# HENDRIX-ZT2/pyaudiorestoration

Measured on AMD Instinct MI355X. Metric: Msamples/sec resampled (192 kHz varispeed), higher is better.
Workload: dtype f32 near taps, far taps (|n| >= 3) as float16 hi + lo x 2^-12 filter banks on v_mfma_f32_16x16x32_f16 with f32 accumulation / f64 positions

## Files before the change

pyaudiorestoration_amd/csrc/sinc2.hip:

```cpp
#define PAR_WANT_BANK2 1
#include "par_common.h"
#include "pos_plan.h"
#include "sinc_taps_gen.h"
#include "sinc_common.h"
#include "sinc_block.h"
#include <algorithm>
#include <atomic>
#include <limits.h>
#include <type_traits>

constexpr int kMaxTilesPerWave = 23;
#ifndef PAR_S2_EXP
#define PAR_S2_EXP 0
#endif

namespace par {

typedef _Float16 half8v __attribute__((ext_vector_type(8)));
typedef _Float16 half2v __attribute__((ext_vector_type(2)));
typedef float float4v __attribute__((ext_vector_type(4)));

constexpr int kRing = 512;
constexpr int kPass = 128;
constexpr float kImgScale = 1024.0f, kImgScaleInv = 0.0009765625f;
constexpr float kImgMax = 32.0f;
constexpr float kQuiet = 0.0001220703125f;


#if PAR_S2_EXP & 64
__device__ unsigned long long* g_s2_phase;
#define S2_MARK(k)                                              \
  do {                                                          \
    const unsigned long long now_ = __builtin_readcyclecounter(); \
    ph_[k] += now_ - pt_;                                       \
    pt_ = now_;                                                 \
  } while (0)
#else
#define S2_MARK(k) do { } while (0)
#endif

struct S2Args {
  int64_t len_out;
  const float* sig;
  int64_t len_in;
  float* out;
  const TileHdr* hdr;
  const BlockRec* rec;
  const BlockRec2* rec2;
  int* redo_count;
  int* redo_list;
  int tiles;
  int tiles_tail;
  int64_t n_big;
  int64_t n_full;
  int64_t n_tiles;
  int n_edge;
  int64_t out_stride;
  FusedArgs fa;
// ... 77 lines not shown
  const bool last = (unsigned)u == ((m >> kRecLastShift) & 63u);
  const float frac = fmaf(u2f, e2, fmaf(uf, e1, F));
  const float e = fmaf(e2, last ? tw0 : tw1, e1);
  const float ri = rintf(frac);
  S2Row o;
  o.s = frac - ri;
  o.c = cbase + irel + (int)ri;
  o.ep = __builtin_amdgcn_fmed3f(e, 0.0f, 3.0e38f);
  o.bad = (m & (kRecSlow0 | kRecSlow1 | kRecCubic)) != 0u || !(fabsf(fabsf(o.s) - 0.5f) > tolf);
  return o;
}


constexpr int kRingF = 1024;
constexpr int kRingH = 512;

template <int NCH, bool MOM = true>
struct S3Lds {
  static constexpr bool kMoments = MOM;
  float ring_head[4 * NCH];
  float ring[kRingF * NCH];
  float ring_tail[4 * NCH];
  _Float16 img[2 * NCH][kRingH];
  float4v qa[kPass];
  float4v qm0[MOM ? kPass : kPass / 4];
  float4v qm1[MOM ? kPass : 1];
  __device__ __forceinline__ float& e2d2(int sl) {
    return MOM ? reinterpret_cast<float*>(&qm0[sl])[3] : reinterpret_cast<float*>(&qm0[0])[sl];
  }
  __device__ __forceinline__ const float& e2d2(int sl) const {
    return MOM ? reinterpret_cast<const float*>(&qm0[sl])[3] : reinterpret_cast<const float*>(&qm0[0])[sl];
  }
#ifdef PAR_S3_LDS_PAD
  uint4 pad[PAR_S3_LDS_PAD / 16];
#endif
  uint4 recs[4][16];
};
static_assert(offsetof(S3Lds<1>, img) % 16 == 0 && offsetof(S3Lds<1>, qa) % 16 == 0 && offsetof(S3Lds<1>, recs) % 16 == 0, "16-byte aligned");
static_assert(offsetof(S3Lds<2>, ring) % 16 == 0 && offsetof(S3Lds<2>, img) % 16 == 0 && offsetof(S3Lds<2>, qa) % 16 == 0 &&
              offsetof(S3Lds<2>, recs) % 16 == 0, "16-byte aligned");
static_assert(sizeof(S3Lds<2>) <= 20480, "eight stereo streams per compute unit (160 KB of LDS)");
using S3LdsUnity = S3Lds<1, false>;
static_assert(sizeof(S3LdsUnity) <= 10240 && offsetof(S3LdsUnity, recs) % 16 == 0 && offsetof(S3LdsUnity, qa) % 16 == 0,
              "sixteen fc = 1 streams per compute unit");

struct S3Pass {
  int c[2];
  float s[2], ep[2];
  int nok[2];
  int j, ws;
};

constexpr int kCtabUnity = 10;
template <bool MOMENTS, bool SIX = true, class LDS>
__device__ __forceinline__ void bank_image3m(LDS& L, const half8v (&fr)[kBank2Frags], const half8v (&fmr)[kBank3Frags],
                                             const int offs, const int l, const int ch = 0) {
  const int bb = l & 15, g = l >> 4;
  const int i0 = offs + 8 * bb + 8 * g;
  half8v xh[3], xl[3];
#pragma unroll
  for (int ks = 0; ks < 3; ++ks) {
    const int ix = (i0 + 32 * ks) & (kRingH - 1);
    xh[ks] = *reinterpret_cast<const half8v*>(&L.img[2 * ch][ix]);
    xl[ks] = *reinterpret_cast<const half8v*>(&L.img[2 * ch + 1][ix]);
  }
  auto frag = [&](int f) { return f < kCtabUnity ? fr[f] : fmr[f - kCtabUnity]; };
  const float4v z = {0.0f, 0.0f, 0.0f, 0.0f};
  float4v e0 = z, lo = z, e1 = z, e2 = z;
#pragma unroll
  for (int ks = 0; ks < 3; ++ks) {
    const half8v f0 = frag(ks);
    e0 = __builtin_amdgcn_mfma_f32_16x16x32_f16(f0, xh[ks], e0, 0, 0, 0);
    lo = __builtin_amdgcn_mfma_f32_16x16x32_f16(frag(5 + ks), xh[ks], lo, 0, 0, 0);
    lo = __builtin_amdgcn_mfma_f32_16x16x32_f16(f0, xl[ks], lo, 0, 0, 0);
    if (ks < 2) {
      const half8v f1 = frag(3 + ks);
      e1 = __builtin_amdgcn_mfma_f32_16x16x32_f16(f1, xh[ks], e1, 0, 0, 0);
      e2 = __builtin_amdgcn_mfma_f32_16x16x32_f16(frag(8 + ks), xh[ks], e2, 0, 0, 0);
    }
  }
  float lo_inv = kBank2LoInv;
  asm volatile("" : "+v"(lo_inv));
  const float4v v0 = e0 + lo * lo_inv, v1 = e1;
  float4v a01 = z, l01 = z, a23 = z, a45 = z, a6 = z;
  if (MOMENTS) {
#pragma unroll
    for (int ks = 0; ks < 3; ++ks) {
      const half8v f01 = frag(kCtabUnity + ks);
      a01 = __builtin_amdgcn_mfma_f32_16x16x32_f16(f01, xh[ks], a01, 0, 0, 0);
      l01 = __builtin_amdgcn_mfma_f32_16x16x32_f16(frag(kCtabUnity + 3 + ks), xh[ks], l01, 0, 0, 0);
      l01 = __builtin_amdgcn_mfma_f32_16x16x32_f16(f01, xl[ks], l01, 0, 0, 0);
      a23 = __builtin_amdgcn_mfma_f32_16x16x32_f16(frag(kCtabUnity + 6 + ks), xh[ks], a23, 0, 0, 0);
      a45 = __builtin_amdgcn_mfma_f32_16x16x32_f16(frag(kCtabUnity + 9 + ks), xh[ks], a45, 0, 0, 0);
      if constexpr (SIX) a6 = __builtin_amdgcn_mfma_f32_16x16x32_f16(frag(kCtabUnity + 12 + ks), xh[ks], a6, 0, 0, 0);
    }
  }
  const float4v m01 = a01 + l01 * lo_inv;
#pragma unroll
  for (int p = 0; p < 2; ++p) {
    const int sl = (8 * bb + 2 * g + p) ^ (bb & 7);
    const float4v row = {v0[2 * p], v0[2 * p + 1], v1[2 * p], v1[2 * p + 1]};
    L.qa[sl] = row;
    const float e2d2 = __uint_as_float(pack_h2(e2[2 * p] * 0.015625f, e2[2 * p + 1] * 0.015625f));
    if constexpr (MOMENTS) {
      const float4v r0 = {m01[2 * p], m01[2 * p + 1], a23[2 * p], e2d2};
      L.qm0[sl] = r0;
      const float4v r1 = {a23[2 * p + 1], a45[2 * p], a45[2 * p + 1], a6[2 * p]};
      L.qm1[sl] = r1;
    } else {
      L.e2d2(sl) = e2d2;
    }
  }
}

template <int MODE, int NCH = 1, class LDS>
__device__ __forceinline__ float s3_out_row(const LDS& L, const int ci, const float sr, const float epr, const int wsK, const int ch = 0) {
  using T32 = TapTab<32>;
  constexpr float kUs = kBank2ScaleInv * kImgScaleInv;
  constexpr float kMs = kImgScaleInv;
  const int sl = ci ^ ((ci >> 3) & 7);
  const int rc = (wsK + ci) & (kRingF - 1);
  const float* xp = &L.ring[NCH * rc + ch];
  const float xm2 = xp[-2 * NCH], xm1 = xp[-NCH], x0 = xp[0], xp1 = xp[NCH], xp2 = xp[2 * NCH];
  const float q = sr * sr, q64 = 64.0f * q;
  const float R1 = fast_rcp(fmaf(q, T32::B[1], T32::A[1])), R2 = fast_rcp(fmaf(q, T32::B[2], T32::A[2]));
  {
    const float E1 = xp1 + xm1, D1 = xp1 - xm1, E2 = xp2 + xm2, D2 = xp2 - xm2;
    const float4v row = L.qa[sl];
    float4v M0 = {0.0f, 0.0f, 0.0f, 0.0f};
    unsigned w2;
    if constexpr (MODE != 1) {
      M0 = L.qm0[sl];
      w2 = __float_as_uint(M0[3]);
    } else {
      w2 = __float_as_uint(L.e2d2(sl));
    }
    const float e = fmaf(q, fmaf(q64, h_lo(w2), row[2]), row[0]), d = fmaf(q, fmaf(q64, h_hi(w2), row[3]), row[1]);
    const float en = fmaf(E2, R2, -(E1 * R1));
    const float dn = fmaf(D2 + D2, R2, -(D1 * R1));
    const float et = fmaf(e, kUs, en), dt = fmaf(d, kUs, dn);
    const float spq = sinpi_poly(q);
    const float unity = spq * fmaf(-sr, fmaf(sr, et, dt), x0 * 0.318309886f);
    if constexpr (MODE == 1) return unity;
    else {
    const float4v Mh = L.qm1[sl];
    const float m3 = Mh[0], m4 = Mh[1], m5 = Mh[2], m6 = Mh[3];
    const float g = epr * fast_rcp(1.0f + epr);
    const float G = 3.14159265f * g, w = G * sr, w2m = w * w, G32 = 32.0f * G;
    float re, im;
    if constexpr (MODE == 3) {
      re = m6 * (1.98412698e-4f * kMs);
      im = 0.0f;
    } else {
      re = m5 * (1.38888889e-3f * kMs);
      im = m5 * (w * -(1.19047619e-3f * kMs));
    }
#define S3_MOM_STEP(Mi, A0, A1, B0)                                   \
    {                                                                 \
      const float al_ = (A1) != 0.0f ? fmaf(w2m, -((A1) * kMs), (A0) * kMs) : (A0) * kMs, be_ = w * -((B0) * kMs);       \
      const float nre_ = fmaf(-G32, im, (Mi) * al_), nim_ = fmaf(G32, re, (Mi) * be_); \
      re = nre_;                                                      \
      im = nim_;                                                      \
    }
    if constexpr (MODE == 3) S3_MOM_STEP(m5, 1.38888889e-3f, 0.0f, 1.19047619e-3f)
    S3_MOM_STEP(m4, 8.33333333e-3f, 0.0f, 6.94444444e-3f)
    S3_MOM_STEP(m3, 4.16666667e-2f, 0.0f, 3.33333333e-2f)
    S3_MOM_STEP(M0[2], 1.66666667e-1f, 5.0e-2f, 1.25e-1f)
    S3_MOM_STEP(M0[1], 0.5f, 0.125f, 3.33333333e-1f)
    S3_MOM_STEP(M0[0], 1.0f, 1.66666667e-1f, 0.5f)
#undef S3_MOM_STEP
    const float S = sr * spq, C = __builtin_amdgcn_cosf(0.5f * sr);
    return fmaf(-g, fmaf(C, re, -(S * im)), unity);
    }
  }
}

template <class LDS>
__device__ __forceinline__ bool s3_convert(LDS& L, const int chunk, const int l) {
  const int wi = chunk * kPass + 2 * l;
  const int ix = wi & (kRingF - 1), ih = wi & (kRingH - 1);
  const float2 xx = *reinterpret_cast<const float2*>(&L.ring[ix]);
  const float x0 = xx.x, x1 = xx.y;
  const float am = fmaxf(fabsf(x0), fabsf(x1));
  const bool ok = !(__ballot(!(fabsf(x0) < kImgMax) || !(fabsf(x1) < kImgMax)) != 0ull ||
                    (__ballot(am >= kQuiet) == 0ull && __ballot(am > 0.0f) != 0ull));
  if ((chunk & 7) == 0 && l < 2) *reinterpret_cast<float2*>(&L.ring_tail[ix]) = xx;
  if ((chunk & 7) == 7 && l == kWave - 1) *reinterpret_cast<float2*>(&L.ring_head[2]) = xx;
  const float s0 = x0 * kImgScale, s1 = x1 * kImgScale;
  const half2v h = {S2_HI(s0), S2_HI(s1)};
  const half2v lo = {(_Float16)((s0 - (float)h[0]) * 4096.0f), (_Float16)((s1 - (float)h[1]) * 4096.0f)};
  *reinterpret_cast<half2v*>(&L.img[0][ih]) = h;
  *reinterpret_cast<half2v*>(&L.img[1][ih]) = lo;
  return ok;
}

template <class LDS>
__device__ __forceinline__ bool s3_convert_ch(LDS& L, const int chunk, const int l, const int ch, const bool mirrors) {
  const int wi = chunk * kPass + 2 * l;
  const int ix = wi & (kRingF - 1), ih = wi & (kRingH - 1);
  const float4v xx = *reinterpret_cast<const float4v*>(&L.ring[2 * ix]);
  const float x0 = ch ? xx[1] : xx[0], x1 = ch ? xx[3] : xx[2];
  const float am = fmaxf(fabsf(x0), fabsf(x1));
  const bool ok = !(__ballot(!(fabsf(x0) < kImgMax) || !(fabsf(x1) < kImgMax)) != 0ull ||
                    (__ballot(am >= kQuiet) == 0ull && __ballot(am > 0.0f) != 0ull));
  if (mirrors) {
    if ((chunk & 7) == 0 && l < 2) *reinterpret_cast<float4v*>(&L.ring_tail[2 * ix]) = xx;
    if ((chunk & 7) == 7 && l == kWave - 1) *reinterpret_cast<float4v*>(&L.ring_head[4]) = xx;
  }
  const float s0 = x0 * kImgScale, s1 = x1 * kImgScale;
  const half2v h = {S2_HI(s0), S2_HI(s1)};
  const half2v lo = {(_Float16)((s0 - (float)h[0]) * 4096.0f), (_Float16)((s1 - (float)h[1]) * 4096.0f)};
  *reinterpret_cast<half2v*>(&L.img[2 * ch][ih]) = h;
  *reinterpret_cast<half2v*>(&L.img[2 * ch + 1][ih]) = lo;
  return ok;
}

constexpr float kEpMaxMom = 0.0125f / (1.0f - 0.0125f);
constexpr float kEpMom5 = 0.0105f / (1.0f - 0.0105f), kEpMom5Lo = 0.95f * kEpMom5;
#ifndef PAR_S3_SHARE_OUT
#define PAR_S3_SHARE_OUT 1
#endif
#ifndef PAR_S3_PIN_MONO
#define PAR_S3_PIN_MONO 0
#endif
template <int NCH, int KIND>
__device__ __forceinline__ void sinc_pipe_body(const S2Args& a, const int bx, S3Lds<NCH, KIND != 1>& L) {
  static_assert(NCH == 1 || NCH == 2, "mono, or an interleaved stereo file");
  static_assert(KIND == 0 || KIND == 3 || NCH == 1, "the stereo form takes every stream");
  static_assert(KIND != 3 || NCH == 2, "one channel of FRAMES");
  constexpr bool kPick = KIND == 3;
  constexpr bool kTwo = NCH == 2 && !kPick;
  constexpr bool kMom = KIND != 1;
  const int l = threadIdx.x & (kWave - 1);
  if (bx < a.n_edge) {
    if constexpr (KIND == 1) return;
    else {
    const int e = bx / kEdgeWavesPerTile, w = bx % kEdgeWavesPerTile;
    const int64_t T = e == 0 ? 0 : a.n_full - 3 + e;
    const int64_t jw = T * kSincTileOutputs + (int64_t)w * kEdgeWaveOut;
    const int nrem = (int)(a.len_out - jw < (int64_t)kEdgeWaveOut ? (a.len_out - jw > 0 ? a.len_out - jw : 0) : kEdgeWaveOut);
    float* const piece = reinterpret_cast<float*>(&L);
    static_assert(sizeof(L) >= fused_capw(2 * NCH, NCH) * NCH * sizeof(float), "the wave's span fits the stream's LDS");
    if constexpr (kPick) {
      static_assert(sizeof(L) >= fused_capw(2, 1) * sizeof(float), "the wave's span fits the stream's LDS");
      if (nrem > 0)
        fused_wave<1, 32, 2, false>(a.len_out, a.sig, nullptr, 2, a.len_in, 32, a.tab, a.tmd, a.out, nullptr, a.out_stride, a.fa, piece, l,
                                    jw, nrem, piece);
      return;
    }
    if (nrem == kEdgeWaveOut)
      fused_wave<NCH, 32, 2 * NCH, true>(a.len_out, a.sig, a.sig + 1, NCH, a.len_in, 32, a.tab, a.tmd, a.out, a.out + 1, NCH, a.fa, piece, l,
                                         jw, nrem, piece);
    else if (nrem > 0)
      fused_wave<NCH, 32, 2 * NCH, false>(a.len_out, a.sig, a.sig + 1, NCH, a.len_in, 32, a.tab, a.tmd, a.out, a.out + 1, NCH, a.fa, piece, l,
                                          jw, nrem, piece);
    return;
    }
  }
  const int64_t stream_id = (int64_t)bx - a.n_edge;
  const int my_tiles = stream_id < a.n_big ? a.tiles : a.tiles_tail;
  const int64_t Ta = stream_id < a.n_big ? stream_id * a.tiles : a.n_big * a.tiles + (stream_id - a.n_big) * a.tiles_tail;
  if (Ta >= a.n_full) return;
  const int64_t Tb = Ta + my_tiles < a.n_full ? Ta + my_tiles : a.n_full;
  const int64_t Ja = Ta * kSincTileOutputs, Jb = Tb * kSincTileOutputs;
  long long A0;
  int hd_dA, hd_fl;
  {
    const int64_t Ti = Ta + l < a.n_tiles ? Ta + l : a.n_tiles - 1;
    const TileHdr h = a.hdr[l <= my_tiles ? Ti : Ta];
    A0 = (long long)(((unsigned long long)(unsigned)__builtin_amdgcn_readfirstlane((int)((unsigned long long)h.anchor >> 32)) << 32) |
                     (unsigned)__builtin_amdgcn_readfirstlane((int)(unsigned)(unsigned long long)h.anchor));
    const long long d = h.anchor - A0;
    hd_fl = h.flags | ((d > -0x40000000ll && d < 0x40000000ll) ? 0 : 1);
    if (a.n_edge > 0 && (Ta + l == 0 || Ta + l >= a.n_full - 2)) hd_fl |= 1 | kTileEdge;
    hd_dA = (int)d;
    if constexpr (KIND == 1 || KIND == 2) {
      const bool any_slow = __ballot(l < my_tiles && Ta + l < Tb && (h.flags & kTileMaySlow) != 0) != 0ull;
      if (any_slow != (KIND == 2)) return;
    }
  }
  half8v fr[kBank2Frags];
  {
    const uint4* src = reinterpret_cast<const uint4*>(kBank2Frags32) + l;
#pragma unroll
    for (int f = 0; f < kBank2Frags; ++f) fr[f] = __builtin_bit_cast(half8v, src[f * kWave]);
// ... 8 lines not shown
    uint4* z = reinterpret_cast<uint4*>(&L.img[0][0]);
    const uint4 zero = {0u, 0u, 0u, 0u};
#pragma unroll
    for (int i = 0; i < (int)(sizeof(L.img) / 16 / kWave); ++i) z[i * kWave + l] = zero;
  }
  const float tolf = (float)((fabs((double)A0) + 2.0e7) * 1.2e-16 + 2.0e-10) + 2.0e-7f;
  const int nJ = (int)(Jb - Ja);
  float* const outW = a.out + (kPick ? a.out_stride : (int64_t)NCH) * Ja;
  const uint4* const recW = reinterpret_cast<const uint4*>(a.rec) + (Ja >> kRecShift);
  const uint4* const rec2W = reinterpret_cast<const uint4*>(a.rec2) + (Ja >> kRecShift);
  const int blk_max = (int)(((a.len_out + kRec - 1) >> kRecShift) - (Ja >> kRecShift)) - 1;

  int j0 = 0;
  int wbase = 0, conv_next = 0, conv_lo = 0, dma_next = 0, dma_bad = INT_MAX, mode = 0, pk = 0;
  int regime = 1;
  int rbA = 0, rbB = 0, rbC = 0;

  const uint4* const rec_lane = (l < 8 ? recW : rec2W) + (l & 7);
  auto fetch_records = [&](int buf, int blk0) {
    if (l < 16) dma_dwordx4(rec_lane + (blk0 < 0 ? 0 : blk0), &L.recs[buf][0]);
  };
  int dma_klo = 0, dma_khi = -1;
  const float* ring_src = a.sig;
  auto ring_restart = [&]() {
    const long long o = A0 + wbase;
    ring_src = a.sig + NCH * o;
    const long long klo = o >= 0 ? 0 : (-o + kPass - 1) / kPass, khi = ((long long)a.len_in - (kPick ? 1 : 0) - o) / kPass - 1;
    dma_klo = (int)(klo > 0x3fffffff ? 0x3fffffff : klo);
    dma_khi = (int)(khi > 0x3fffffff ? 0x3fffffff : (khi < -1 ? -1 : khi));
  };
  const unsigned lane_bytes = 4u * (unsigned)l;
  auto chunk_dma = [&](int k) {
    const bool inside = k >= dma_klo && k <= dma_khi;
    if (!inside) dma_bad = k < dma_bad ? k : dma_bad;
    const float* src = inside ? ring_src + (long long)(kPass * NCH) * k : a.sig;
    if constexpr (NCH == 2) dma_chunk256(src, lane_bytes, &L.ring[(k & 7) * (kPass * 2)]);
    else dma_chunk128(src, lane_bytes, &L.ring[(k & 7) * kPass]);
  };
  auto push_tile = [&](int64_t T) {
    if (l == 0) {
      const int slot = atomicAdd(a.redo_count, 1);
      a.redo_list[slot] = (int)T;
    }
  };
  if (stream_id == 0 && a.n_full < a.n_tiles && a.n_edge == 0) push_tile(a.n_full);

  struct Placed {
    S2Row R[2];
    int nt[2];
    int fl0, fl1, tend;
    int epm;
  };
  int tc_T = -1, tc_dA0 = 0, tc_dA1 = 0, tc_fl0 = 0, tc_fl1 = 0;
  auto place = [&](int j, int buf, int rb) {
    Placed P;
    const int T = j >> 10;
    P.tend = (T + 1) << 10;
    if (T != tc_T) {
      tc_T = T;
      tc_dA0 = __builtin_amdgcn_readlane(hd_dA, T);
      tc_dA1 = __builtin_amdgcn_readlane(hd_dA, T + 1);
      tc_fl0 = __builtin_amdgcn_readlane(hd_fl, T);
      tc_fl1 = __builtin_amdgcn_readlane(hd_fl, T + 1);
    }
    const int dA0 = tc_dA0, dA1 = tc_dA1;
    P.fl0 = tc_fl0;
    P.fl1 = tc_fl1;
    const int t5 = (j & (kRec - 1)) + l;
    const int u = t5 & (kRec - 1);
    const int bi = ((j >> kRecShift) - rb + (t5 >> kRecShift)) & 7;
    const uint4* rp = &L.recs[buf][0];
    const uint4 ra0 = rp[bi], rb0 = rp[8 + bi], ra1 = rp[(bi + 2) & 7], rb1 = rp[8 + ((bi + 2) & 7)];
    const int uc = u - kRec / 2;
    const float uf = (float)uc, u2f = uf * uf, tw1 = fmaf(2.0f, uf, 1.0f), tw0 = tw1 - 2.0f;
    P.nt[0] = clamp64(P.tend - j);
    P.nt[1] = clamp64(P.tend - j - 64);
    if (__ballot((unsigned)u > (ra0.x & 31u) || (unsigned)u > (ra1.x & 31u)) == 0ull) {
      P.R[0] = s2_place_row<false>(ra0, rb0, u, (l < P.nt[0] ? dA0 : dA1) + uc, uf, u2f, tw1, tw0, tolf);
      P.R[1] = s2_place_row<false>(ra1, rb1, u, (l < P.nt[1] ? dA0 : dA1) + uc, uf, u2f, tw1, tw0, tolf);
    } else {
      P.R[0] = s2_place_row(ra0, rb0, u, (l < P.nt[0] ? dA0 : dA1) + uc, uf, u2f, tw1, tw0, tolf);
      P.R[1] = s2_place_row(ra1, rb1, u, (l < P.nt[1] ? dA0 : dA1) + uc, uf, u2f, tw1, tw0, tolf);
    }
    P.epm = max(__float_as_int(P.R[0].ep), __float_as_int(P.R[1].ep));
    return P;
  };

  S3Pass P;
  P.nok[0] = P.nok[1] = 0;
  P.j = P.ws = 0;
  P.c[0] = P.c[1] = 0;
  P.s[0] = P.s[1] = P.ep[0] = P.ep[1] = 0.0f;

  auto out_pass = [&](auto mode_tag, const S3Pass& Q, float (&res)[2], const int ch = 0) {
    constexpr int MODE = decltype(mode_tag)::value;
    const int wsK = Q.ws - wbase;
#pragma unroll
    for (int r = 0; r < 2; ++r) {
      int ci = Q.c[r] - Q.ws;
      ci = ci < 0 ? 0 : (ci > kPass - 1 ? kPass - 1 : ci);
      float sr = Q.s[r], epr = Q.ep[r];
#if !PAR_S3_SHARE_OUT
      if (NCH == 2 && ch == 1) asm volatile("" : "+v"(sr), "+v"(epr));
#endif
      res[r] = s3_out_row<MODE, NCH>(L, ci, sr, epr, wsK, ch);
    }
  };
  auto store_pass = [&](const S3Pass& Q, const float (&res)[2]) {
#pragma unroll
    for (int r = 0; r < 2; ++r)
      if (l < Q.nok[r] && !(PAR_S2_EXP & 4)) {
        if constexpr (kPick) outW[(int64_t)((unsigned)Q.j + 64u * r + (unsigned)l) * a.out_stride] = res[r];
        else outW[(unsigned)Q.j + 64u * r + (unsigned)l] = res[r];
      }
  };
  auto store_pass2 = [&](const S3Pass& Q, const float (&res0)[2], const float (&res1)[2]) {
#pragma unroll
    for (int r = 0; r < 2; ++r)
      if (l < Q.nok[r] && !(PAR_S2_EXP & 4))
        reinterpret_cast<float2*>(outW)[(unsigned)Q.j + 64u * r + (unsigned)l] = make_float2(res0[r], res1[r]);
  };
  auto convert_chunk = [&](int chunk) -> bool {
    if constexpr (kPick) {
      return s3_convert_ch(L, chunk, l, 0, true);
    } else if constexpr (NCH == 2) {
      const bool ok0 = s3_convert_ch(L, chunk, l, 0, true);
      const bool ok1 = s3_convert_ch(L, chunk, l, 1, false);
      return ok0 && ok1;
    } else {
      return s3_convert(L, chunk, l);
    }
  };

#if PAR_S2_EXP & 128
#define S3_COUNT(k) do { if (l == 0) atomicAdd(a.redo_count + (k), 1); } while (0)
#else
#define S3_COUNT(k) do { } while (0)
#endif
  auto start_run = [&]() -> bool {
// ... 107 lines not shown
      float res[2];
      if (kMom && regime == 3) out_pass(std::integral_constant<int, kMom ? 3 : 1>{}, N, res);
      else if (kMom && regime == 2) out_pass(std::integral_constant<int, kMom ? 2 : 1>{}, N, res);
      else out_pass(std::integral_constant<int, 1>{}, N, res);
      if constexpr (kTwo) {
        float res1[2];
        wave_lds_fence();
        if (regime == 3) bank_image3m<true, true>(L, fr, fmr, offs, l, 1);
        else if (regime == 2) bank_image3m<true, false>(L, fr, fmr, offs, l, 1);
        else bank_image3m<false>(L, fr, fmr, offs, l, 1);
        wave_lds_fence();
        if (regime == 3) out_pass(std::integral_constant<int, 3>{}, N, res1, 1);
        else if (regime == 2) out_pass(std::integral_constant<int, 2>{}, N, res1, 1);
        else out_pass(std::integral_constant<int, 1>{}, N, res1, 1);
        store_pass2(N, res, res1);
      } else {
        store_pass(N, res);
      }
    }
  };

#if PAR_S2_EXP & 64
  unsigned long long s3t_[4] = {0, 0, 0, 0}, s3last_ = __builtin_readcyclecounter();
  const unsigned long long s3start_ = s3last_;
#endif
  auto hot = [&](auto mode_tag) {
    constexpr int MODE = decltype(mode_tag)::value;
    j0 = __builtin_amdgcn_readfirstlane(j0);
    wbase = __builtin_amdgcn_readfirstlane(wbase);
    conv_next = __builtin_amdgcn_readfirstlane(conv_next);
    dma_next = __builtin_amdgcn_readfirstlane(dma_next);
    dma_bad = __builtin_amdgcn_readfirstlane(dma_bad);
    pk = __builtin_amdgcn_readfirstlane(pk);
    rbA = __builtin_amdgcn_readfirstlane(rbA);
    rbB = __builtin_amdgcn_readfirstlane(rbB);
    rbC = __builtin_amdgcn_readfirstlane(rbC);
    for (;;) {
#if PAR_S2_EXP & 64
      const unsigned long long tA_ = __builtin_readcyclecounter();
#endif
      if constexpr (NCH == 2) asm volatile("s_waitcnt vmcnt(7)" ::: "memory");
      else asm volatile("s_waitcnt vmcnt(5)" ::: "memory");
#if PAR_S2_EXP & 64
      const unsigned long long tB_ = __builtin_readcyclecounter();
      s3t_[0] += tB_ - tA_;
      s3t_[1] += tA_ - s3last_;
      s3last_ = tB_;
      s3t_[2] += 1;
#endif
      wave_lds_fence();
      S3Pass N;
      bool ok;
      int wsK;
      auto place_next = [&]() {
      const Placed Q = place(j0, pk & 3, rbA);
      const unsigned long long bad = __ballot(Q.R[0].bad || Q.R[1].bad || Q.epm > __float_as_int(kEpMaxMom));
      const unsigned long long gen = __ballot(Q.epm > 0x33800000);
      bool tier = true;
      if constexpr (MODE == 2) tier = __ballot(Q.epm > __float_as_int(kEpMom5)) == 0ull;
      if constexpr (MODE == 3) tier = __ballot(Q.epm > __float_as_int(kEpMom5Lo)) != 0ull;
      const int ws = __builtin_amdgcn_readfirstlane(Q.R[0].c) & ~7;
#pragma unroll
      for (int r = 0; r < 2; ++r) {
        N.c[r] = Q.R[r].c;
        N.s[r] = Q.R[r].s;
        N.ep[r] = Q.R[r].ep;
        N.nok[r] = __popcll(__ballot(Q.R[r].c - ws < kPass));
      }
      N.j = j0;
      N.ws = ws;
      wsK = ws - wbase;
      const int d = kPass * conv_next - wsK;
      ok = (((Q.fl0 | Q.fl1) & 1) == 0) & (bad == 0ull) & (j0 + kPass <= nJ) & (N.nok[0] + N.nok[1] >= 120) &
           (MODE == 1 ? gen == 0ull : gen != 0ull) & tier & ((unsigned)(d - 161) <= 312u) & (conv_next + 1 < dma_bad) &
           ((unsigned)((j0 >> kRecShift) - rbA) <= 1u);
      };
      if constexpr (!kTwo) place_next();
      float res[2];
      out_pass(mode_tag, P, res);
      bool cok;
      if constexpr (kTwo) {
        float res1[2];
        asm volatile("" : "+v"(res[0]), "+v"(res[1]));
        bank_image3m<MODE != 1, MODE == 3>(L, fr, fmr, P.ws - wbase - 31, l, 1);
        out_pass(mode_tag, P, res1, 1);
        asm volatile("" : "+v"(res1[0]), "+v"(res1[1]));
        place_next();
        const int offs = wsK - 31;
        bank_image3m<MODE != 1, MODE == 3>(L, fr, fmr, offs, l, 0);
        const bool c0 = s3_convert_ch(L, conv_next, l, 0, true);
        const bool c1 = s3_convert_ch(L, conv_next - 1, l, 1, false);
        cok = c0 && c1;
        fetch_records((pk + 2) & 3, rbC);
        chunk_dma(dma_next);
        store_pass2(P, res, res1);
      } else {
        const int offs = wsK - 31;
#if PAR_S3_PIN_MONO
        asm volatile("" : "+v"(res[0]), "+v"(res[1]));
#endif
        bank_image3m<MODE != 1, MODE == 3>(L, fr, fmr, offs, l);
        cok = convert_chunk(conv_next);
        fetch_records((pk + 2) & 3, rbC);
        chunk_dma(dma_next);
        store_pass(P, res);
      }
      wave_lds_fence();
      ++conv_next;
      ++dma_next;
      if (!cok) mode = 0;
      S3_COUNT(2);
#if PAR_S2_EXP & 128
      if (!(ok && cok)) {
        if (((Q.fl0 | Q.fl1) & 1) != 0 || bad != 0ull) S3_COUNT(3);
        else if (!(j0 + kPass <= nJ)) S3_COUNT(4);
        else if (!(N.nok[1] >= 1 && N.nok[0] + N.nok[1] >= 120)) S3_COUNT(5);
        else if (!(MODE == 1 ? gen == 0ull : gen != 0ull)) S3_COUNT(6);
        else if (!(d >= 161 && d <= 473)) S3_COUNT(7);
        else if (!(conv_next < dma_bad)) S3_COUNT(9);
        else if (!((unsigned)((j0 >> kRecShift) - rbA) <= 1u)) S3_COUNT(11);
        else if (!cok) S3_COUNT(10);
        else S3_COUNT(8);
      }
#endif
      if (!(ok && cok)) {
        if constexpr (kTwo)
          if (mode != 0 && !s3_convert_ch(L, conv_next - 1, l, 1, false)) mode = 0;
        return;
      }
      P = N;
      j0 += N.nok[0] + N.nok[1];
      ++pk;
      rbA = rbB;
      rbB = rbC;
      rbC = (j0 + 240) >> kRecShift;
    }
  };

  while (start_run()) {
    if (kMom && regime == 3) hot(std::integral_constant<int, kMom ? 3 : 1>{});
    else if (kMom && regime == 2) hot(std::integral_constant<int, kMom ? 2 : 1>{});
    else hot(std::integral_constant<int, 1>{});
  }
  __builtin_amdgcn_s_waitcnt(0x0F70);
#if PAR_S2_EXP & 64
  if (l == 0) {
    unsigned long long* o = g_s2_phase + (size_t)stream_id * 16;
    o[0] = s3t_[0];
    o[1] = s3t_[1];
    o[2] = s3t_[2];
    o[3] = __builtin_readcyclecounter() - s3start_;
    o[6] = s3t_[2];
  }
#endif
}

template <int NCH, int KIND>
__global__ __launch_bounds__(kWave, KIND == 1 ? 3 : 2) void k_sinc_pipe(const S2Args a) {
// ... 116 lines not shown
```

pyaudiorestoration_amd/csrc/sinc_block.h:

```cpp
#pragma once
#include "par_common.h"
#include "pos_plan.h"
#include "sinc_taps_gen.h"
#include "sinc_common.h"
#include <atomic>
#include <utility>
#include <limits.h>
#include <math.h>
#include <map>
#include <vector>

#ifndef PAR_SINC_EXP
#define PAR_SINC_EXP 0
#endif
#ifndef PAR_SINC_HOT
#define PAR_SINC_HOT 1
#endif
#ifndef PAR_SINC_WAVES
#define PAR_SINC_WAVES 6
#endif
#ifndef PAR_FARROW_BARRIER_EARLY
#define PAR_FARROW_BARRIER_EARLY 0
#endif
#ifndef PAR_MFMA_EXP
// ... 75 lines not shown
  for (long long k0 = 0; k0 < L; k0 += kSlowChunk) {
    float xs[kSlowChunk];
#pragma unroll
    for (int u = 0; u < kSlowChunk; ++u) xs[u] = k0 + u < L ? sig[(lower + k0 + u) * sig_stride] : 0.0f;
#pragma unroll
    for (int u = 0; u < kSlowChunk; ++u) {
      const long long k = k0 + u;
      if (k >= L) break;
      double x = ((double)(k - NT) - shift) * fc;
      x = x == 0.0 ? 1e-20 : x;
      double si = sinpi_f64(x) / (M_PI * x) * fc;
      float win = (float)(0.5 + 0.5 * sinpi_f64((double)(k - NT) / (double)NT + 0.5));
      acc += (double)xs[u] * si * (double)win;
    }
  }
  return (float)acc;
}

__device__ __noinline__ float2 sinc_two_f64(double p, double dp, const float* __restrict__ sig, const float* __restrict__ sig1,
                                            int64_t sig_stride, int64_t len_in, int NT) {
  if (!(fabs(p) < 9.0e18)) return make_float2(0.0f, 0.0f);
  const long long ind = llrint(p);
  const long long lower = ind - NT > 0 ? ind - NT : 0;
  const long long upper = ind + NT < (long long)len_in ? ind + NT : (long long)len_in;
  const long long L = upper - lower;
  if (L <= 0) return make_float2(0.0f, 0.0f);
  const double period = dp > 1e-12 ? dp : 1e-12;
  const double inv = 1.0 / period;
  const double fc = inv < 1.0 ? inv : 1.0;
  const double shift = p - (double)ind;
  double acc0 = 0.0, acc1 = 0.0;
  for (long long k0 = 0; k0 < L; k0 += kSlowChunk) {
    float xs[kSlowChunk], ys[kSlowChunk];
#pragma unroll
    for (int u = 0; u < kSlowChunk; ++u) {
      xs[u] = k0 + u < L ? sig[(lower + k0 + u) * sig_stride] : 0.0f;
      ys[u] = k0 + u < L ? sig1[(lower + k0 + u) * sig_stride] : 0.0f;
    }
#pragma unroll
    for (int u = 0; u < kSlowChunk; ++u) {
      const long long k = k0 + u;
      if (k >= L) break;
      double x = ((double)(k - NT) - shift) * fc;
      x = x == 0.0 ? 1e-20 : x;
      const double si = sinpi_f64(x) / (M_PI * x) * fc;
      const float win = (float)(0.5 + 0.5 * sinpi_f64((double)(k - NT) / (double)NT + 0.5));
      acc0 += (double)xs[u] * si * (double)win;
      acc1 += (double)ys[u] * si * (double)win;
    }
  }
  return make_float2((float)acc0, (float)acc1);
}

template <int NCH>
__device__ __noinline__ float2 sinc_slow_wave(bool want, double p, double dp, const float* __restrict__ sig,
                                              const float* __restrict__ sig1, int64_t sig_stride, int64_t len_in, int NT, int l) {
  const unsigned long long mask = __ballot(want);
  const int n = __popcll(mask);
  int sh = 0;
  while ((n << (sh + 1)) <= kWave) ++sh;
  const int f = 1 << sh, g = l >> sh, sub = l & (f - 1);
  unsigned long long rest = mask;
  for (int i = 0; i < g && rest; ++i) rest &= rest - 1;
  const bool active = g < n;
  const int src = rest ? __builtin_ctzll(rest) : 0;
  const double pg = __shfl(p, src, kWave), dpg = __shfl(dp, src, kWave);
  double acc0 = 0.0, acc1 = 0.0;
  if (active && fabs(pg) < 9.0e18) {
    const long long ind = llrint(pg);
    const long long lower = ind - NT > 0 ? ind - NT : 0;
    const long long upper = ind + NT < (long long)len_in ? ind + NT : (long long)len_in;
    const long long L = upper - lower;
    const double period = dpg > 1e-12 ? dpg : 1e-12;
    const double inv = 1.0 / period;
    const double fc = inv < 1.0 ? inv : 1.0;
    const double shift = pg - (double)ind;
    for (long long k = sub; k < L; k += f) {
      double x = ((double)(k - NT) - shift) * fc;
      x = x == 0.0 ? 1e-20 : x;
      const double si = sinpi_f64(x) / (M_PI * x) * fc;
      const float win = (float)(0.5 + 0.5 * sinpi_f64((double)(k - NT) / (double)NT + 0.5));
      acc0 += (double)sig[(lower + k) * sig_stride] * si * (double)win;
      if (NCH == 2) acc1 += (double)sig1[(lower + k) * sig_stride] * si * (double)win;
    }
  }
  for (int o = f >> 1; o > 0; o >>= 1) {
    acc0 += __shfl_xor(acc0, o, kWave);
    if (NCH == 2) acc1 += __shfl_xor(acc1, o, kWave);
  }
  const int rank = __popcll(mask & ((1ull << l) - 1ull));
  const int from = want ? (rank << sh) : l;
  const double r0 = __shfl(acc0, from, kWave), r1 = NCH == 2 ? __shfl(acc1, from, kWave) : 0.0;
  return make_float2((float)r0, (float)r1);
}

constexpr int kChunk = 4;
typedef __attribute__((address_space(3))) const float lds_cfloat;
#ifndef PAR_SINC_OPAQUE
#define PAR_SINC_OPAQUE 1
#endif
template <bool OPQ>
__device__ __forceinline__ lds_cfloat* opaque_lds(lds_cfloat* p) {
  if (!PAR_SINC_OPAQUE || !OPQ) return p;
  unsigned a = (unsigned)(uintptr_t)p;
  asm("" : "+v"(a));
  return (lds_cfloat*)(uintptr_t)a;
}

// ... 540 lines not shown

template <int NT, int R, int LS = 1, bool OPQ = false>
__device__ __forceinline__ void taps_unity_near(const float* __restrict__ tile, const int (&c)[R], const float (&s)[R],
                                                const float (&q)[R], const float (&far)[R], float (&res)[R]) {
  using T = TapTab<NT>;
  lds_cfloat* tl = (lds_cfloat*)tile;
  constexpr float b0 = T::B[0];
#pragma unroll
  for (int r = 0; r < R; ++r) {
    lds_cfloat* base = opaque_lds<OPQ>(tl + c[r] - NT * LS);
    float e0 = fmaf(base[0], 0.0f, 0.0f), d0 = 0.0f;
    static_for<kPoly2From - 1>([&](auto idx) {
#pragma clang fp contract(off)
      constexpr int n = 1 + decltype(idx)::value;
      static_assert(T::mode[n] == kRcp, "reciprocal rows");
      constexpr float fn = (float)n;
      const float sp = base[(NT + n) * LS], sm = base[(NT - n) * LS];
      const float D = sp - sm, E = sp + sm;
      const float x = q[r] * T::B[n] + T::A[n];
      const float Rn = fast_rcp(x);
      const float DR = D * Rn;
      if constexpr (n & 1) {
        e0 = fmaf(-E, Rn, e0);
        d0 = fmaf(DR, -fn, d0);
      } else {
        e0 = fmaf(E, Rn, e0);
        d0 = fmaf(DR, fn, d0);
      }
    });
    const float centre = tile[c[r]] * fast_rcp(s[r] * b0);
    res[r] = -sinpi_half(s[r]) * (centre + fmaf(far[r], FarGeom<NT == 50 ? 50 : 32>::kScaleInv, fmaf(s[r], e0, d0)));
  }
}


__device__ __forceinline__ void place_from_pos(double p, double dp, double anchor_d, int& c, float& s, float& fc, float& dd,
                                               bool& lowfc, bool& wild) {
  const double rel = p - anchor_d;
  const double rf = rint(rel);
  wild = !(fabs(rel) < 1.0e9);
  c = wild ? 0 : (int)rf;
  const float sh = (float)(rel - rf);
  s = (sh == 0.0f) ? 1e-20f : sh;
  const bool one = !(dp > 1.0);
  lowfc = dp > 8.0;
  const float inv = fast_rcp((float)(dp > 1e-12 ? dp : 1e-12));
  fc = one ? 1.0f : inv;
  dd = one ? 0.0f : (float)(dp - 1.0) * inv;
}

struct PosDp {
  double p, dp;
};
__device__ __noinline__ PosDp place_exact(const double* __restrict__ speeds, const int64_t* __restrict__ seg_start,
                                          const double* __restrict__ seg_off, const double* __restrict__ ckp, long long i,
                                          long long j, long long len_out) {
#pragma clang fp contract(off)
  const long long start = seg_start[i], n = seg_start[i + 1] - start;
  const long long k = j - start, b = ckp ? k / kCk : 0;
  const Ramp r = make_ramp(speeds[i], speeds[i + 1], n);
  const double off = seg_off[i];
  double c = b ? ckp[ck_slot0(start, i) + b] : 0.0;
  double cprev = c;
  long long v = b * kCk;
  for (; v + 8 <= k + 1; v += 8) {
    double rr[8];
#pragma unroll
    for (int u = 0; u < 8; ++u) rr[u] = ramp_recip((double)(v + u), r);
#pragma unroll
    for (int u = 0; u < 8; ++u) {
      cprev = c;
      c = c + rr[u];
    }
  }
  for (; v <= k; ++v) {
    cprev = c;
    c = c + ramp_recip((double)v, r);
  }
  PosDp o;
  o.p = c + off;
  if (j + 1 < len_out) {
    double pn;
    if (k + 1 < n) {
      pn = (c + ramp_recip((double)(k + 1), r)) + off;
    } else {
      const long long n2 = seg_start[i + 2] - seg_start[i + 1];
      const Ramp r2 = make_ramp(speeds[i + 1], speeds[i + 2], n2);
      pn = (0.0 + ramp_recip(0.0, r2)) + seg_off[i + 1];
    }
    o.dp = pn - o.p;
  } else {
    const double pp = k > 0 ? cprev + off : off;
    o.dp = o.p - pp;
  }
  return o;
}

__device__ __forceinline__ void place_fast(const FusedArgs& fa, long long i, long long j, long long len_out, long long anchor,
                                           double tol, int& c, float& s, float& fc, float& dd, bool& lowfc, bool& wild,
                                           bool& exact, const bool lazy) {
  const long long start = fa.seg_start[i];
  const SegFast sf = fa.seg_fast[i];
  const double s0 = fa.speeds[i];
  const int k = (int)(j - start);
  const int u = lazy ? k : (k & (kCk - 1));
  const long long b = lazy ? 0 : (k >> 3);
  static_assert(kCk == 8, "k >> 3");
// ... 592 lines not shown
```

Baseline: 170,500.

## Split LDS loads from math and hoist pass loads ahead of MFMA work

Splits the bank image, output row, convert and record-placement steps into separate load and math halves. An optional mono path, off by default behind PAR_S3_EARLY_LDS, issues all LDS reads for the next pass before any arithmetic, with scheduling barriers, so LDS latency overlaps the MFMA and FMA work. Separately, and active by default, the cold fallbacks sinc_slow_wave and place_exact are force-inlined in this kernel instead of being out-of-line calls. That removes call and ABI overhead but can raise register pressure and code size.

```diff
diff --git a/pyaudiorestoration_amd/csrc/sinc2.hip b/pyaudiorestoration_amd/csrc/sinc2.hip
--- a/pyaudiorestoration_amd/csrc/sinc2.hip
+++ b/pyaudiorestoration_amd/csrc/sinc2.hip
@@ -3,7 +3,11 @@
 #include "pos_plan.h"
 #include "sinc_taps_gen.h"
 #include "sinc_common.h"
+#define PAR_COLD_FN __forceinline__
 #include "sinc_block.h"
+#ifndef PAR_COLD_FN_GIVEN
+#error "sinc_block.h was included before PAR_COLD_FN was defined: the cold functions would stay out of line"
+#endif
 #include <algorithm>
 #include <atomic>
 #include <limits.h>
@@ -187,18 +191,27 @@
 };
 
 constexpr int kCtabUnity = 10;
-template <bool MOMENTS, bool SIX = true, class LDS>
-__device__ __forceinline__ void bank_image3m(LDS& L, const half8v (&fr)[kBank2Frags], const half8v (&fmr)[kBank3Frags],
-                                             const int offs, const int l, const int ch = 0) {
+struct S3Frags {
+  half8v xh[3], xl[3];
+};
+template <class LDS>
+__device__ __forceinline__ S3Frags bank_load(const LDS& L, const int offs, const int l, const int ch = 0) {
   const int bb = l & 15, g = l >> 4;
   const int i0 = offs + 8 * bb + 8 * g;
-  half8v xh[3], xl[3];
+  S3Frags X;
 #pragma unroll
   for (int ks = 0; ks < 3; ++ks) {
     const int ix = (i0 + 32 * ks) & (kRingH - 1);
-    xh[ks] = *reinterpret_cast<const half8v*>(&L.img[2 * ch][ix]);
-    xl[ks] = *reinterpret_cast<const half8v*>(&L.img[2 * ch + 1][ix]);
-  }
+    X.xh[ks] = *reinterpret_cast<const half8v*>(&L.img[2 * ch][ix]);
+    X.xl[ks] = *reinterpret_cast<const half8v*>(&L.img[2 * ch + 1][ix]);
+  }
+  return X;
+}
+template <bool MOMENTS, bool SIX = true, class LDS>
+__device__ __forceinline__ void bank_math(LDS& L, const half8v (&fr)[kBank2Frags], const half8v (&fmr)[kBank3Frags],
+                                          const S3Frags& X, const int l) {
+  const int bb = l & 15, g = l >> 4;
+  const half8v (&xh)[3] = X.xh, (&xl)[3] = X.xl;
   auto frag = [&](int f) { return f < kCtabUnity ? fr[f] : fmr[f - kCtabUnity]; };
   const float4v z = {0.0f, 0.0f, 0.0f, 0.0f};
   float4v e0 = z, lo = z, e1 = z, e2 = z;
@@ -247,29 +260,47 @@
     }
   }
 }
-
+template <bool MOMENTS, bool SIX = true, class LDS>
+__device__ __forceinline__ void bank_image3m(LDS& L, const half8v (&fr)[kBank2Frags], const half8v (&fmr)[kBank3Frags],
+                                             const int offs, const int l, const int ch = 0) {
+  bank_math<MOMENTS, SIX>(L, fr, fmr, bank_load(L, offs, l, ch), l);
+}
+
+struct S3Gather {
+  float4v row, M0, Mh;
+  float xm2, xm1, x0, xp1, xp2;
+};
 template <int MODE, int NCH = 1, class LDS>
-__device__ __forceinline__ float s3_out_row(const LDS& L, const int ci, const float sr, const float epr, const int wsK, const int ch = 0) {
+__device__ __forceinline__ S3Gather s3_out_load(const LDS& L, const int ci, const int wsK, const int ch = 0) {
+  const int sl = ci ^ ((ci >> 3) & 7);
+  const int rc = (wsK + ci) & (kRingF - 1);
+  const float* xp = &L.ring[NCH * rc + ch];
+  S3Gather G;
+  G.xm2 = xp[-2 * NCH], G.xm1 = xp[-NCH], G.x0 = xp[0], G.xp1 = xp[NCH], G.xp2 = xp[2 * NCH];
+  G.row = L.qa[sl];
+  G.M0 = float4v{0.0f, 0.0f, 0.0f, 0.0f};
+  G.Mh = G.M0;
+  if constexpr (MODE != 1) {
+    G.M0 = L.qm0[sl];
+    G.Mh = L.qm1[sl];
+  } else {
+    G.M0[3] = L.e2d2(sl);
+  }
+  return G;
+}
+template <int MODE>
+__device__ __forceinline__ float s3_out_math(const S3Gather& Gr, const float sr, const float epr) {
   using T32 = TapTab<32>;
   constexpr float kUs = kBank2ScaleInv * kImgScaleInv;
   constexpr float kMs = kImgScaleInv;
-  const int sl = ci ^ ((ci >> 3) & 7);
-  const int rc = (wsK + ci) & (kRingF - 1);
-  const float* xp = &L.ring[NCH * rc + ch];
-  const float xm2 = xp[-2 * NCH], xm1 = xp[-NCH], x0 = xp[0], xp1 = xp[NCH], xp2 = xp[2 * NCH];
+  const float xm2 = Gr.xm2, xm1 = Gr.xm1, x0 = Gr.x0, xp1 = Gr.xp1, xp2 = Gr.xp2;
   const float q = sr * sr, q64 = 64.0f * q;
   const float R1 = fast_rcp(fmaf(q, T32::B[1], T32::A[1])), R2 = fast_rcp(fmaf(q, T32::B[2], T32::A[2]));
   {
     const float E1 = xp1 + xm1, D1 = xp1 - xm1, E2 = xp2 + xm2, D2 = xp2 - xm2;
-    const float4v row = L.qa[sl];
-    float4v M0 = {0.0f, 0.0f, 0.0f, 0.0f};
-    unsigned w2;
-    if constexpr (MODE != 1) {
-      M0 = L.qm0[sl];
-      w2 = __float_as_uint(M0[3]);
-    } else {
-      w2 = __float_as_uint(L.e2d2(sl));
-    }
+    const float4v row = Gr.row;
+    const float4v M0 = Gr.M0;
+    const unsigned w2 = __float_as_uint(M0[3]);
     const float e = fmaf(q, fmaf(q64, h_lo(w2), row[2]), row[0]), d = fmaf(q, fmaf(q64, h_hi(w2), row[3]), row[1]);
     const float en = fmaf(E2, R2, -(E1 * R1));
     const float dn = fmaf(D2 + D2, R2, -(D1 * R1));
@@ -278,7 +309,7 @@
     const float unity = spq * fmaf(-sr, fmaf(sr, et, dt), x0 * 0.318309886f);
     if constexpr (MODE == 1) return unity;
     else {
-    const float4v Mh = L.qm1[sl];
+    const float4v Mh = Gr.Mh;
     const float m3 = Mh[0], m4 = Mh[1], m5 = Mh[2], m6 = Mh[3];
     const float g = epr * fast_rcp(1.0f + epr);
     const float G = 3.14159265f * g, w = G * sr, w2m = w * w, G32 = 32.0f * G;
@@ -309,12 +340,20 @@
     }
   }
 }
+template <int MODE, int NCH = 1, class LDS>
+__device__ __forceinline__ float s3_out_row(const LDS& L, const int ci, const float sr, const float epr, const int wsK, const int ch = 0) {
+  return s3_out_math<MODE>(s3_out_load<MODE, NCH>(L, ci, wsK, ch), sr, epr);
+}
 
 template <class LDS>
-__device__ __forceinline__ bool s3_convert(LDS& L, const int chunk, const int l) {
+__device__ __forceinline__ float2 s3_convert_load(const LDS& L, const int chunk, const int l) {
+  const int ix = (chunk * kPass + 2 * l) & (kRingF - 1);
+  return *reinterpret_cast<const float2*>(&L.ring[ix]);
+}
+template <class LDS>
+__device__ __forceinline__ bool s3_convert_math(LDS& L, const int chunk, const int l, const float2 xx) {
   const int wi = chunk * kPass + 2 * l;
   const int ix = wi & (kRingF - 1), ih = wi & (kRingH - 1);
-  const float2 xx = *reinterpret_cast<const float2*>(&L.ring[ix]);
   const float x0 = xx.x, x1 = xx.y;
   const float am = fmaxf(fabsf(x0), fabsf(x1));
   const bool ok = !(__ballot(!(fabsf(x0) < kImgMax) || !(fabsf(x1) < kImgMax)) != 0ull ||
@@ -328,6 +367,10 @@
   *reinterpret_cast<half2v*>(&L.img[1][ih]) = lo;
   return ok;
 }
+template <class LDS>
+__device__ __forceinline__ bool s3_convert(LDS& L, const int chunk, const int l) {
+  return s3_convert_math(L, chunk, l, s3_convert_load(L, chunk, l));
+}
 
 template <class LDS>
 __device__ __forceinline__ bool s3_convert_ch(LDS& L, const int chunk, const int l, const int ch, const bool mirrors) {
@@ -358,6 +401,9 @@
 #ifndef PAR_S3_PIN_MONO
 #define PAR_S3_PIN_MONO 0
 #endif
+#ifndef PAR_S3_EARLY_LDS
+#define PAR_S3_EARLY_LDS 0
+#endif
 template <int NCH, int KIND>
 __device__ __forceinline__ void sinc_pipe_body(const S2Args& a, const int bx, S3Lds<NCH, KIND != 1>& L) {
   static_assert(NCH == 1 || NCH == 2, "mono, or an interleaved stereo file");
@@ -366,6 +412,7 @@
   constexpr bool kPick = KIND == 3;
   constexpr bool kTwo = NCH == 2 && !kPick;
   constexpr bool kMom = KIND != 1;
+  constexpr bool kEarly = NCH == 1 && ((KIND == 2 && (PAR_S3_EARLY_LDS & 1)) || (KIND == 1 && (PAR_S3_EARLY_LDS & 2) == 2));
   const int l = threadIdx.x & (kWave - 1);
   if (bx < a.n_edge) {
     if constexpr (KIND == 1) return;
@@ -480,7 +527,16 @@
     int epm;
   };
   int tc_T = -1, tc_dA0 = 0, tc_dA1 = 0, tc_fl0 = 0, tc_fl1 = 0;
-  auto place = [&](int j, int buf, int rb) {
+  struct PlaceRecs {
+    uint4 ra0, rb0, ra1, rb1;
+  };
+  auto place_load = [&](int j, int buf, int rb) {
+    const int t5 = (j & (kRec - 1)) + l;
+    const int bi = ((j >> kRecShift) - rb + (t5 >> kRecShift)) & 7;
+    const uint4* rp = &L.recs[buf][0];
+    return PlaceRecs{rp[bi], rp[8 + bi], rp[(bi + 2) & 7], rp[8 + ((bi + 2) & 7)]};
+  };
+  auto place_impl = [&](int j, int buf, int rb, auto early, const PlaceRecs& RR) {
     Placed P;
     const int T = j >> 10;
     P.tend = (T + 1) << 10;
@@ -496,9 +552,14 @@
     P.fl1 = tc_fl1;
     const int t5 = (j & (kRec - 1)) + l;
     const int u = t5 & (kRec - 1);
-    const int bi = ((j >> kRecShift) - rb + (t5 >> kRecShift)) & 7;
-    const uint4* rp = &L.recs[buf][0];
-    const uint4 ra0 = rp[bi], rb0 = rp[8 + bi], ra1 = rp[(bi + 2) & 7], rb1 = rp[8 + ((bi + 2) & 7)];
+    uint4 ra0, rb0, ra1, rb1;
+    if constexpr (decltype(early)::value) {
+      ra0 = RR.ra0, rb0 = RR.rb0, ra1 = RR.ra1, rb1 = RR.rb1;
+    } else {
+      const int bi = ((j >> kRecShift) - rb + (t5 >> kRecShift)) & 7;
+      const uint4* rp = &L.recs[buf][0];
+      ra0 = rp[bi], rb0 = rp[8 + bi], ra1 = rp[(bi + 2) & 7], rb1 = rp[8 + ((bi + 2) & 7)];
+    }
     const int uc = u - kRec / 2;
     const float uf = (float)uc, u2f = uf * uf, tw1 = fmaf(2.0f, uf, 1.0f), tw0 = tw1 - 2.0f;
     P.nt[0] = clamp64(P.tend - j);
@@ -513,6 +574,7 @@
     P.epm = max(__float_as_int(P.R[0].ep), __float_as_int(P.R[1].ep));
     return P;
   };
+  auto place = [&](int j, int buf, int rb) { return place_impl(j, buf, rb, std::false_type{}, PlaceRecs{}); };
 
   S3Pass P;
   P.nok[0] = P.nok[1] = 0;
@@ -726,8 +788,8 @@
       S3Pass N;
       bool ok;
       int wsK;
-      auto place_next = [&]() {
-      const Placed Q = place(j0, pk & 3, rbA);
+      auto place_next = [&](auto early, const PlaceRecs& RR) {
+      const Placed Q = place_impl(j0, pk & 3, rbA, early, RR);
       const unsigned long long bad = __ballot(Q.R[0].bad || Q.R[1].bad || Q.epm > __float_as_int(kEpMaxMom));
       const unsigned long long gen = __ballot(Q.epm > 0x33800000);
       bool tier = true;
@@ -749,17 +811,46 @@
            (MODE == 1 ? gen == 0ull : gen != 0ull) & tier & ((unsigned)(d - 161) <= 312u) & (conv_next + 1 < dma_bad) &
            ((unsigned)((j0 >> kRecShift) - rbA) <= 1u);
       };
-      if constexpr (!kTwo) place_next();
       float res[2];
+      bool cok;
+      if constexpr (kEarly) {
+        const PlaceRecs RR = place_load(j0, pk & 3, rbA);
+        const float2 cxx = s3_convert_load(L, conv_next, l);
+        S3Gather G[2];
+        const int wsP = P.ws - wbase;
+#pragma unroll
+        for (int r = 0; r < 2; ++r) {
+          int ci = P.c[r] - P.ws;
+          ci = ci < 0 ? 0 : (ci > kPass - 1 ? kPass - 1 : ci);
+          G[r] = s3_out_load<MODE, NCH>(L, ci, wsP);
+        }
+        __builtin_amdgcn_sched_barrier(0);
+        place_next(std::true_type{}, RR);
+        const S3Frags X = bank_load(L, wsK - 31, l);
+        __builtin_amdgcn_sched_barrier(0);
+#pragma unroll
+        for (int r = 0; r < 2; ++r) res[r] = s3_out_math<MODE>(G[r], P.s[r], P.ep[r]);
+        asm volatile("" : "+v"(res[0]), "+v"(res[1]));
+        if constexpr (MODE == 2) asm volatile("" ::"v"(G[0].Mh[3]), "v"(G[1].Mh[3]));
+        __builtin_amdgcn_sched_barrier(0);
+        bank_math<MODE != 1, MODE == 3>(L, fr, fmr, X, l);
+        int oki = __builtin_amdgcn_readfirstlane((int)ok);
+        asm volatile("" : "+s"(oki));
+        ok = oki != 0;
+        cok = s3_convert_math(L, conv_next, l, cxx);
+        fetch_records((pk + 2) & 3, rbC);
+        chunk_dma(dma_next);
+        store_pass(P, res);
+      } else {
+      if constexpr (!kTwo) place_next(std::false_type{}, PlaceRecs{});
       out_pass(mode_tag, P, res);
-      bool cok;
       if constexpr (kTwo) {
         float res1[2];
         asm volatile("" : "+v"(res[0]), "+v"(res[1]));
         bank_image3m<MODE != 1, MODE == 3>(L, fr, fmr, P.ws - wbase - 31, l, 1);
         out_pass(mode_tag, P, res1, 1);
         asm volatile("" : "+v"(res1[0]), "+v"(res1[1]));
-        place_next();
+        place_next(std::false_type{}, PlaceRecs{});
         const int offs = wsK - 31;
         bank_image3m<MODE != 1, MODE == 3>(L, fr, fmr, offs, l, 0);
         const bool c0 = s3_convert_ch(L, conv_next, l, 0, true);
@@ -778,6 +869,7 @@
         fetch_records((pk + 2) & 3, rbC);
         chunk_dma(dma_next);
         store_pass(P, res);
+      }
       }
       wave_lds_fence();
       ++conv_next;
diff --git a/pyaudiorestoration_amd/csrc/sinc_block.h b/pyaudiorestoration_amd/csrc/sinc_block.h
--- a/pyaudiorestoration_amd/csrc/sinc_block.h
+++ b/pyaudiorestoration_amd/csrc/sinc_block.h
@@ -151,8 +151,13 @@
   return make_float2((float)acc0, (float)acc1);
 }
 
+#ifdef PAR_COLD_FN
+#define PAR_COLD_FN_GIVEN 1
+#else
+#define PAR_COLD_FN __noinline__
+#endif
 template <int NCH>
-__device__ __noinline__ float2 sinc_slow_wave(bool want, double p, double dp, const float* __restrict__ sig,
+__device__ PAR_COLD_FN float2 sinc_slow_wave(bool want, double p, double dp, const float* __restrict__ sig,
                                               const float* __restrict__ sig1, int64_t sig_stride, int64_t len_in, int NT, int l) {
   const unsigned long long mask = __ballot(want);
   const int n = __popcll(mask);
@@ -799,7 +804,7 @@
 struct PosDp {
   double p, dp;
 };
-__device__ __noinline__ PosDp place_exact(const double* __restrict__ speeds, const int64_t* __restrict__ seg_start,
+__device__ PAR_COLD_FN PosDp place_exact(const double* __restrict__ speeds, const int64_t* __restrict__ seg_start,
                                           const double* __restrict__ seg_off, const double* __restrict__ ckp, long long i,
                                           long long j, long long len_out) {
 #pragma clang fp contract(off)
```

Result: faster. 172,300, median of 6 (+1.1%).
